# yeyupiaoling/VoiceprintRecognition-Pytorch

Measured on NVIDIA H100. Metric: embeddings/sec (3s@16kHz) ECAPA-TDNN, higher is better.
Workload: dtype f32

## Files before the change

### voiceprintrecognition-pytorch_b200/csrc/api.cu

```cuda
#include <cmath>
#include <cstdarg>
#include <cstdio>
#include <cstdlib>
#include <cstring>
#include <new>
#include <string>
#include <vector>

#include "kernels.cuh"


using namespace vpb;

struct vp_handle {
  int device = 0;
  std::string err;
  float* d_weights = nullptr;
  size_t weights_bytes = 0;
  char* d_arena = nullptr;
  size_t arena_bytes = 0;
  cudaStream_t cap_stream = nullptr;
  bool fe_set = false;
  vp_frontend_desc fe{};
  float* d_window = nullptr;
  double2* d_twiddle = nullptr;
  int* d_mel_start = nullptr;
  int* d_mel_count = nullptr;
  int* d_mel_off = nullptr;
  float* d_mel_w = nullptr;
  float* d_dct = nullptr;
};

struct vp_program {
  vp_handle* h = nullptr;
  std::vector<vp_op> ops;
  std::vector<int> engines;
  size_t ws_bytes = 0, in_floats = 0, out_floats = 0;
  int launches = 0;
  int B = 0;
  cudaGraphExec_t gexec = nullptr;
  const float* g_feats = nullptr;
  float* g_emb = nullptr;
  char* g_arena = nullptr;
  int runs = 0, g_miss = 0;
  bool g_off = false;
  int n_slots = 0;
  size_t arena_need() const { return ws_bytes + (((size_t)n_slots * 4 + 255) & ~(size_t)255); }
  unsigned* slot(int32_t q) const { return q > 0 ? reinterpret_cast<unsigned*>(h->d_arena + ws_bytes) + (q - 1) : nullptr; }
};

static int fail(vp_handle* h, int code, const char* fmt, ...) {
  char buf[512];
  va_list ap;
  va_start(ap, fmt);
  vsnprintf(buf, sizeof(buf), fmt, ap);
  va_end(ap);
  if (h) h->err = buf;
  return code;
}
#define CUDA_TRY(h, expr)                                                                          \
  do {                                                                                             \
    cudaError_t e__ = (expr);                                                                      \
    if (e__ != cudaSuccess) return fail(h, VP_ERR_CUDA, "%s: %s", #expr, cudaGetErrorString(e__)); \
  } while (0)

static const int FPB = 16;

static bool tc16_enabled() {
  static int on = -1;
  if (on < 0) { const char* e = getenv("VPB_TC_F16"); on = (e && e[0] == '0') ? 0 : 1; }
  return on == 1;
}

extern "C" {

static void fill_conv(const vp_program* p, const vp_op& o, const float* feats, float* emb, vpb::ConvParams& c);

int vp_abi_version(void) { return VP_ABI_VERSION; }
int32_t vp_sizeof_op(void) { return (int32_t)sizeof(vp_op); }
int32_t vp_sizeof_frontend_desc(void) { return (int32_t)sizeof(vp_frontend_desc); }

int vp_create(int device, vp_handle** out) {
  if (!out) return VP_ERR_INVALID;
  *out = nullptr;
  int n = 0;
  cudaError_t e = cudaGetDeviceCount(&n);
  if (e != cudaSuccess || device < 0 || device >= n) return VP_ERR_CUDA;
  cudaDeviceProp prop;
  if (cudaGetDeviceProperties(&prop, device) != cudaSuccess) return VP_ERR_CUDA;
// ... 295 lines not shown
      const long long rows = (long long)o.B * o.Tin;
      TRY(check_act_buf(p, "x", o.src, view_floats(rows, o.in_ld, o.in_coff, o.Cin), false, i));
      TRY(check_act_buf(p, "logits", o.src2, view_floats(rows, o.src2_ld, o.src2_coff, o.Cin), false, i));
      if (o.mode != 0 && o.mode != 1) return fail(h, VP_ERR_INVALID, "op %d: asp mode", i);
      TRY(check_act_buf(p, "dst", o.dst, view_floats(o.B, o.out_ld, o.out_coff, (o.mode == 1 ? 1 : 2) * o.Cin), true, i));
      return VP_OK;
    }
    case VP_OP_POOL2D: {
      if (o.Tin < 1 || o.Fin < 1 || o.Tout < 1 || o.Fout < 1 || o.KT < 1 || o.KF < 1 || o.sT < 1 || o.sF < 1 || o.padT < 0 ||
          o.padF < 0 || o.Cin < 4 || (o.Cin & 3) || (o.in_ld & 3) || (o.in_coff & 3) || (o.out_ld & 3) || (o.out_coff & 3) ||
          (o.mode != 0 && o.mode != 1))
        return fail(h, VP_ERR_INVALID, "op %d: pool geometry / alignment", i);
      if ((long long)(o.Tout - 1) * o.sT - o.padT >= o.Tin || (long long)(o.Fout - 1) * o.sF - o.padF >= o.Fin ||
          o.padT >= o.KT || o.padF >= o.KF)
        return fail(h, VP_ERR_INVALID, "op %d: pooling window entirely outside the map", i);
      TRY(check_act_buf(p, "src", o.src, view_floats((long long)o.B * o.Tin * o.Fin, o.in_ld, o.in_coff, o.Cin), false, i));
      TRY(check_act_buf(p, "dst", o.dst, view_floats((long long)o.B * o.Tout * o.Fout, o.out_ld, o.out_coff, o.Cin), true, i));
      return VP_OK;
    }
    case VP_OP_EW: {
      const long long rows = (long long)o.B * o.Tin * o.Fin;
      if (o.mode == VP_EW_PAD_COPY) {
        if (rows < 1 || o.Cin < 1 || o.Cout < o.Cin || (o.Cout & 3) || (o.out_ld & 3) || (o.out_coff & 3))
          return fail(h, VP_ERR_UNSUPPORTED, "op %d: PAD_COPY shape", i);
        TRY(check_act_buf(p, "x", o.src, view_floats(rows, o.in_ld, o.in_coff, o.Cin), false, i));
        TRY(check_act_buf(p, "dst", o.dst, view_floats(rows, o.out_ld, o.out_coff, o.Cout), true, i));
        return VP_OK;
      }
      if (rows < 1 || o.Cin < 4 || (o.Cin & 3) || (o.in_ld & 3) || (o.in_coff & 3) || (o.out_ld & 3) || (o.out_coff & 3))
        return fail(h, VP_ERR_UNSUPPORTED, "op %d: EW alignment", i);
      if (!act_ok(o.act2)) return fail(h, VP_ERR_INVALID, "op %d: activation id", i);
      TRY(check_act_buf(p, "x", o.src, view_floats(rows, o.in_ld, o.in_coff, o.Cin), false, i));
      TRY(check_act_buf(p, "dst", o.dst, view_floats(rows, o.out_ld, o.out_coff, o.Cin), true, i));
      if (o.mode == VP_EW_GATE_RES) {
        if (o.gate != VP_BUF_NONE) TRY(check_act_buf(p, "gate", o.gate, (size_t)o.B * o.Cin, false, i));
        if (o.res != VP_BUF_NONE) {
          if ((o.res_ld & 3) || (o.res_coff & 3)) return fail(h, VP_ERR_UNSUPPORTED, "op %d: res alignment", i);
          TRY(check_act_buf(p, "res", o.res, view_floats(rows, o.res_ld, o.res_coff, o.Cin), false, i));
        }
      } else if (o.mode == VP_EW_AFF) {
        if ((o.src2_ld & 3) || (o.src2_coff & 3) || (o.res_ld & 3) || (o.res_coff & 3)) return fail(h, VP_ERR_UNSUPPORTED, "op %d: AFF alignment", i);
        TRY(check_act_buf(p, "y", o.src2, view_floats(rows, o.src2_ld, o.src2_coff, o.Cin), false, i));
        TRY(check_act_buf(p, "att", o.res, view_floats(rows, o.res_ld, o.res_coff, o.Cin), false, i));
      } else if (o.mode != VP_EW_COPY) {
        return fail(h, VP_ERR_INVALID, "op %d: EW mode", i);
      }
      return VP_OK;
    }
    default:
      return fail(h, VP_ERR_INVALID, "op %d: unknown kind %d", i, o.kind);
  }
}

int vp_program_create(vp_handle* h, const vp_op* ops, int32_t n_ops, size_t ws_bytes, size_t in_floats,
                      size_t out_floats, vp_program** out) {
  if (!h || !ops || n_ops < 1 || !out) return fail(h, VP_ERR_INVALID, "null/empty program");
  if (!h->d_weights) return fail(h, VP_ERR_INVALID, "load weights before creating a program");
  *out = nullptr;
  vp_program* p = new (std::nothrow) vp_program();
  if (!p) return fail(h, VP_ERR_NOMEM, "host alloc");
  p->h = h;
  p->ops.assign(ops, ops + n_ops);
  p->ws_bytes = (ws_bytes + 255) & ~(size_t)255;
  p->in_floats = in_floats;
  p->out_floats = out_floats;
  p->B = p->ops[0].B;
  for (int i = 0; i < n_ops; ++i)
    if (p->ops[i].src == VP_BUF_INPUT) { p->B = p->ops[i].B; break; }
  for (int i = 0; i < n_ops; ++i) {
    int r = validate_op(p, p->ops[i], i);
    if (r != VP_OK) { delete p; return r; }
  }
  p->launches = n_ops;
  p->engines.assign(n_ops, 0);
  for (int i = 0; i < n_ops; ++i) {
    const vp_op& o = p->ops[i];
    if (o.amax_out > p->n_slots) p->n_slots = o.amax_out;
    if (o.amax_in > p->n_slots) p->n_slots = o.amax_in;
  }
  if (p->n_slots > 0) ++p->launches;
  for (int i = 0; i < n_ops; ++i) {
    const vp_op& o = p->ops[i];
    if (o.kind != VP_OP_CONV) continue;
    ConvParams c;
    fill_conv(p, o, nullptr, nullptr, c);
    c.amax_in = o.amax_in > 0 ? reinterpret_cast<const unsigned*>(8) : nullptr;
    const bool ok = conv_tc_supported(c);
    bool ok16 = ok && o.w_tc16_q > 0 && o.tc16_descale > 0.f && conv_tc16_supported(c);
    if (ok16) {
      const int bn = o.tc_bn, nt = (o.Cout + bn - 1) / bn, kb = (c.K + 63) / 64;
      const size_t off = (size_t)(o.w_tc16_q - 1) << 4, bytes = (size_t)nt * kb * 2 * bn * 128;
      if (off + bytes > h->weights_bytes) {
        int r = fail(h, VP_ERR_INVALID, "op %d: fp16 weight image out of range", i);
        delete p;
        return r;
      }
    }
    if ((o.engine == VP_ENGINE_TC && !ok) || (o.engine == VP_ENGINE_TC16 && !ok16)) {
      int r = fail(h, VP_ERR_UNSUPPORTED, "op %d: shape / operands not supported by the requested tensor-core engine", i);
      delete p;
      return r;
    }
    if (o.engine == VP_ENGINE_TC16 || (o.engine == VP_ENGINE_AUTO && ok16 && tc16_enabled())) p->engines[i] = VP_ENGINE_TC16;
    else if (o.engine == VP_ENGINE_TC || (o.engine == VP_ENGINE_AUTO && ok)) p->engines[i] = VP_ENGINE_TC;
    else p->engines[i] = VP_ENGINE_FFMA;
  }
  if (cudaSetDevice(h->device) != cudaSuccess) { delete p; return fail(h, VP_ERR_CUDA, "cudaSetDevice"); }
  if (p->arena_need() > h->arena_bytes) {
    const size_t want = p->arena_need() + (p->arena_need() >> 3);
    cudaDeviceSynchronize();
    cudaFree(h->d_arena);
    h->d_arena = nullptr;
    h->arena_bytes = 0;
    if (cudaMalloc(&h->d_arena, want) != cudaSuccess) {
      cudaGetLastError();
      if (cudaMalloc(&h->d_arena, p->arena_need()) != cudaSuccess) {
        delete p;
        return fail(h, VP_ERR_NOMEM, "workspace of %zu bytes: %s", ws_bytes, cudaGetErrorString(cudaGetLastError()));
      }
      h->arena_bytes = p->arena_need();
    } else {
      h->arena_bytes = want;
    }
  }
  *out = p;
  return VP_OK;
}

void vp_program_destroy(vp_program* p) {
  if (!p) return;
  if (p->gexec) cudaGraphExecDestroy(p->gexec);
  delete p;
}

size_t vp_workspace_bytes(const vp_handle* h) { return h ? h->arena_bytes : 0; }

int32_t vp_program_launches(const vp_program* p) { return p ? p->launches : -1; }

static inline const float* rd(const vp_program* p, int64_t off, const float* in, const float* out) {
  if (off == VP_BUF_NONE) return nullptr;
  if (off == VP_BUF_INPUT) return in;
  if (off == VP_BUF_OUTPUT) return out;
  return reinterpret_cast<const float*>(p->h->d_arena + off);
}
static inline const float* wt(const vp_program* p, int64_t off) {
  return off < 0 ? nullptr : reinterpret_cast<const float*>(reinterpret_cast<const char*>(p->h->d_weights) + off);
}

static void fill_conv(const vp_program* p, const vp_op& o, const float* feats, float* emb, ConvParams& c) {
  c.src = rd(p, o.src, feats, emb);
  c.src2 = o.src2_mode == VP_SRC2_NONE ? nullptr : rd(p, o.src2, feats, emb);
  c.dst = const_cast<float*>(rd(p, o.dst, feats, emb));
  c.sum = const_cast<float*>(rd(p, o.sum, feats, emb)); c.sum_ld = o.sum_ld; c.sum_coff = o.sum_coff;
  c.res = rd(p, o.res, feats, emb); c.gate = rd(p, o.gate, feats, emb); c.ubias = rd(p, o.ubias, feats, emb);
  c.w = wt(p, o.w); c.w_tc = wt(p, o.w_tc); c.tc_bn = o.tc_bn; c.tc_kc = o.tc_kc; c.bias = wt(p, o.bias); c.pre_s = wt(p, o.pre_s); c.pre_h = wt(p, o.pre_h);
  c.post_s = wt(p, o.post_s); c.post_h = wt(p, o.post_h);
  c.B = o.B; c.Tin = o.Tin; c.Fin = o.Fin; c.Cin = o.Cin;
  c.CinTot = o.Cin + (o.src2_mode == VP_SRC2_CONCAT ? o.Cin2 : 0);
  c.in_ld = o.in_ld; c.in_coff = o.in_coff;
  c.src2_mode = o.src2_mode; c.src2_ld = o.src2_ld; c.src2_coff = o.src2_coff;
  c.Tout = o.Tout; c.Fout = o.Fout; c.out_ld = o.out_ld; c.out_coff = o.out_coff;
  c.res_ld = o.res_ld; c.res_coff = o.res_coff;
  c.KT = o.KT; c.KF = o.KF; c.sT = o.sT; c.sF = o.sF; c.dT = o.dT; c.dF = o.dF; c.padT = o.padT; c.padF = o.padF;
  c.pad_mode = o.pad_mode; c.w_ld = o.w_ld; c.pre_relu = o.pre_relu; c.act = o.act; c.act2 = o.act2;
  c.seg_len = o.seg_len; c.n_seg = o.n_seg;
  c.M = o.B * o.Tout * o.Fout; c.N = o.Cout; c.K = o.KT * o.KF * c.CinTot;
  c.amax_out = p->h->d_arena ? p->slot(o.amax_out) : nullptr;
  c.amax_in = p->h->d_arena ? p->slot(o.amax_in) : nullptr;
}

static int run_ops(vp_program* p, const float* feats, float* emb, cudaStream_t st, cudaEvent_t* evs) {
  vp_handle* h = p->h;
  if (p->n_slots > 0) CUDA_TRY(h, cudaMemsetAsync(h->d_arena + p->ws_bytes, 0, (size_t)p->n_slots * 4, st));
  for (size_t i = 0; i < p->ops.size(); ++i) {
    const vp_op& o = p->ops[i];
    if (evs) CUDA_TRY(h, cudaEventRecord(evs[i], st));
    switch (o.kind) {
      case VP_OP_CONV:
      case VP_OP_CONV_C1: {
        ConvParams c;
        fill_conv(p, o, feats, emb, c);
        if (o.kind == VP_OP_CONV_C1) {
          CUDA_TRY(h, launch_conv_c1(c, st));
        } else {
          if (p->engines[i] == VP_ENGINE_TC16)
            CUDA_TRY(h, launch_conv_tc16(c, reinterpret_cast<const float*>(reinterpret_cast<const char*>(h->d_weights) + ((size_t)(o.w_tc16_q - 1) << 4)),
                                         o.tc16_descale, st));
          else if (p->engines[i] == VP_ENGINE_TC) CUDA_TRY(h, launch_conv_tc(c, st));
          else CUDA_TRY(h, launch_conv_ffma(c, st));
        }
        break;
      }
      case VP_OP_COLSTATS: {
        StatsParams s;
        s.src = rd(p, o.src, feats, emb); s.dst = const_cast<float*>(rd(p, o.dst, feats, emb));
        s.B = o.B; s.R = o.Tin * o.Fin; s.C = o.Cin; s.in_ld = o.in_ld; s.in_coff = o.in_coff;
        s.out_ld = o.out_ld; s.out_coff = o.out_coff; s.mode = o.mode; s.seg_len = o.seg_len; s.n_seg = o.n_seg;
        s.eps = o.eps;
        CUDA_TRY(h, launch_colstats(s, st));
        break;
      }
      case VP_OP_ASP_POOL: {
        AspParams a;
        a.x = rd(p, o.src, feats, emb); a.logit = rd(p, o.src2, feats, emb);
        a.dst = const_cast<float*>(rd(p, o.dst, feats, emb));
        a.B = o.B; a.T = o.Tin; a.C = o.Cin; a.x_ld = o.in_ld; a.x_coff = o.in_coff; a.l_ld = o.src2_ld;
        a.l_coff = o.src2_coff; a.out_ld = o.out_ld; a.out_coff = o.out_coff; a.eps = o.eps; a.mean_only = o.mode == 1;
        CUDA_TRY(h, launch_asp_pool(a, st));
        break;
      }
      case VP_OP_POOL2D: {
        PoolParams q;
        q.src = rd(p, o.src, feats, emb); q.dst = const_cast<float*>(rd(p, o.dst, feats, emb));
        q.B = o.B; q.Tin = o.Tin; q.Fin = o.Fin; q.Tout = o.Tout; q.Fout = o.Fout; q.C = o.Cin;
        q.in_ld = o.in_ld; q.in_coff = o.in_coff; q.out_ld = o.out_ld; q.out_coff = o.out_coff;
        q.KT = o.KT; q.KF = o.KF; q.sT = o.sT; q.sF = o.sF; q.padT = o.padT; q.padF = o.padF; q.mode = o.mode;
        q.amax_out = p->slot(o.amax_out);
        CUDA_TRY(h, launch_pool2d(q, st));
        break;
      }
      case VP_OP_EW: {
        EwParams e;
        e.x = rd(p, o.src, feats, emb);
        e.y = o.mode == VP_EW_AFF ? rd(p, o.src2, feats, emb) : nullptr;
        e.att = o.mode == VP_EW_AFF ? rd(p, o.res, feats, emb) : nullptr;
        e.gate = o.mode == VP_EW_GATE_RES ? rd(p, o.gate, feats, emb) : nullptr;
        e.res = o.mode == VP_EW_GATE_RES ? rd(p, o.res, feats, emb) : nullptr;
        e.dst = const_cast<float*>(rd(p, o.dst, feats, emb));
        e.rows = (long long)o.B * o.Tin * o.Fin; e.C = o.Cin; e.rows_per_utt = o.Tin * o.Fin;
// ... 196 lines not shown
```

### voiceprintrecognition-pytorch_b200/csrc/conv_tc.cu

```cuda
#include <cuda_fp16.h>

#include <cstdlib>
#include <type_traits>

#include "kernels.cuh"
#include "wgmma.cuh"

namespace vpb {

namespace tc {

constexpr int BM = 128;
constexpr int BK = 32;
constexpr int A_TILE = BM * BK * 4;
constexpr int CONSUMER_WARPS = 8;
constexpr int CONSUMER_THREADS = CONSUMER_WARPS * 32;
constexpr int PRODUCER_WARPS = 8;
constexpr int PRODUCER_THREADS = PRODUCER_WARPS * 32;
constexpr int NUM_THREADS = CONSUMER_THREADS + PRODUCER_THREADS;
constexpr int ROWS_PER_THREAD = BM * 8 / PRODUCER_THREADS;
constexpr int MAX_BN = 128;
constexpr int MAX_BN_CHUNKED = 64;
constexpr int SMEM_BUDGET = 225 * 1024;

__device__ __forceinline__ uint32_t smem_u32(const void* p) { return (uint32_t)__cvta_generic_to_shared(p); }

__device__ __forceinline__ void mbar_init(uint32_t bar, uint32_t count) {
  asm volatile("mbarrier.init.shared::cta.b64 [%0], %1;" ::"r"(bar), "r"(count));
}
__device__ __forceinline__ void mbar_arrive(uint32_t bar) {
  asm volatile("mbarrier.arrive.shared::cta.b64 _, [%0];" ::"r"(bar) : "memory");
}
__device__ __forceinline__ void mbar_expect_tx(uint32_t bar, uint32_t bytes) {
  asm volatile("mbarrier.arrive.expect_tx.shared::cta.b64 _, [%0], %1;" ::"r"(bar), "r"(bytes) : "memory");
}
__device__ __forceinline__ void mbar_wait(uint32_t bar, uint32_t parity) {
  asm volatile(
      "{\n\t.reg .pred p;\n\t"
      "WAIT_%=:\n\t"
      "mbarrier.try_wait.parity.shared::cta.b64 p, [%0], %1;\n\t"
      "@p bra DONE_%=;\n\t"
      "bra WAIT_%=;\n\t"
      "DONE_%=:\n\t}" ::"r"(bar), "r"(parity)
      : "memory");
}
__device__ __forceinline__ void bulk_copy_g2s(uint32_t dst, const void* src, uint32_t bytes, uint32_t bar) {
  asm volatile("cp.async.bulk.shared::cluster.global.mbarrier::complete_tx::bytes [%0], [%1], %2, [%3];" ::"r"(dst),
               "l"(src), "r"(bytes), "r"(bar)
               : "memory");
}
__device__ __forceinline__ void fence_proxy_async() { asm volatile("fence.proxy.async.shared::cta;" ::: "memory"); }

__device__ __forceinline__ void wgmma_fence() { asm volatile("wgmma.fence.sync.aligned;" ::: "memory"); }
__device__ __forceinline__ void wgmma_commit() { asm volatile("wgmma.commit_group.sync.aligned;" ::: "memory"); }
template <int N>
__device__ __forceinline__ void wgmma_wait() { asm volatile("wgmma.wait_group.sync.aligned %0;" ::"n"(N) : "memory"); }
template <int N>
__device__ __forceinline__ void fence_regs(float (&d)[N]) {
#pragma unroll
  for (int i = 0; i < N; ++i) asm volatile("" : "+f"(d[i])::"memory");
}

__device__ __forceinline__ uint64_t smem_desc(uint32_t addr) {
  return (uint64_t)((addr >> 4) & 0x3FFF) | (1ull << 16) | (64ull << 32) | (1ull << 62);
}
__device__ __forceinline__ float tf32_rna(float x) {
  uint32_t r;
  asm("cvt.rna.tf32.f32 %0, %1;" : "=r"(r) : "f"(x));
  return __uint_as_float(r);
}

template <int BN, bool F16>
__device__ __forceinline__ void mma_tile(float* d, uint32_t a, uint32_t b, uint32_t scale_d) {
  const uint64_t da = smem_desc(a);
  if constexpr (BN == 128) {
    if constexpr (F16) wgmma_f16_n128(d, da, smem_desc(b), scale_d);
    else wgmma_tf32_n128(d, da, smem_desc(b), scale_d);
  } else {
    constexpr int o64 = 0, o32 = o64 + (BN & 64), o16 = o32 + (BN & 32);
    if constexpr ((BN & 64) != 0) {
      if constexpr (F16) wgmma_f16_n64(d + o64 / 2, da, smem_desc(b + o64 * 128), scale_d);
      else wgmma_tf32_n64(d + o64 / 2, da, smem_desc(b + o64 * 128), scale_d);
    }
    if constexpr ((BN & 32) != 0) {
      if constexpr (F16) wgmma_f16_n32(d + o32 / 2, da, smem_desc(b + o32 * 128), scale_d);
      else wgmma_tf32_n32(d + o32 / 2, da, smem_desc(b + o32 * 128), scale_d);
    }
    if constexpr ((BN & 16) != 0) {
      if constexpr (F16) wgmma_f16_n16(d + o16 / 2, da, smem_desc(b + o16 * 128), scale_d);
      else wgmma_tf32_n16(d + o16 / 2, da, smem_desc(b + o16 * 128), scale_d);
    }
  }
}

__device__ __noinline__ float2 act2_slow(float2 v, int act) {
  v.x = apply_act(v.x, act); v.y = apply_act(v.y, act);
  return v;
}

template <int MODE> struct Slot;
template <> struct Slot<0> { float4 v[ROWS_PER_THREAD]; };
template <> struct Slot<1> { float4 v[ROWS_PER_THREAD]; float4 u[ROWS_PER_THREAD]; };
template <> struct Slot<2> { float4 v[ROWS_PER_THREAD]; float4 ps, ph; uint32_t okmask; };
struct SlotH { float4 v[ROWS_PER_THREAD]; float4 w[ROWS_PER_THREAD]; };

struct TcArgs {
  const float* w_tc;
  int BN;
  int stages;
  int m_tiles, n_tiles, k_blocks;
  int kc, n_chunks;
  int debug;
  float descale;
};

template <int MODE, bool F16, int BN>
__global__ void __launch_bounds__(NUM_THREADS, 1) conv_tc_kernel(const __grid_constant__ ConvParams p,
                                                                 const __grid_constant__ TcArgs a) {
  static_assert(!F16 || MODE == 0, "the fp16 split path only implements the plain / concat source mode");
  static_assert(BN % 16 == 0 && BN >= 16 && BN <= MAX_BN, "N tile");
  constexpr bool CHUNKABLE = BN <= MAX_BN_CHUNKED;
  constexpr int BKE = F16 ? 64 : BK;
  constexpr int KPT = F16 ? 8 : 4;
// ... 451 lines not shown
```

### voiceprintrecognition-pytorch_b200/csrc/kernels.cuh

```cuda
#pragma once
#include "common.cuh"

namespace vpb {

struct FrontendParams {
  const float* wave; float* feats; float* partial;
  const float* window; const double2* twiddle;
  const int* mel_start; const int* mel_count; const int* mel_off; const float* mel_w;
  int B, L, T, kind, N, WL, hop, F, remove_dc, power, use_log, fpb, nblk;
  float preemph, log_floor, db_mult;
  float* cta_max;
  int n_pass, radix[12], G;
};
void frontend_plan(FrontendParams& p);

struct MfccParams {
  const float* mel; const float* cta_max; const float* dct; float* feats; float* partial;
  int B, T, M, K, fpb, nblk, n_max;
  float top_db;
};

struct StatsParams {
  const float* src; float* dst;
  int B, R, C, in_ld, in_coff, out_ld, out_coff, mode, seg_len, n_seg;
// ... 1 lines not shown
};

struct AspParams {
  const float* x; const float* logit; float* dst;
  int B, T, C, x_ld, x_coff, l_ld, l_coff, out_ld, out_coff, mean_only;
  float eps;
};

struct EwParams {
  const float* x; const float* y; const float* att; const float* gate; const float* res; float* dst;
  long long rows; int C, rows_per_utt;
  int x_ld, x_coff, y_ld, y_coff, att_ld, att_coff, res_ld, res_coff, out_ld, out_coff, mode, act2;
  int C_out;
  unsigned* amax_out;
};

struct PoolParams {
  const float* src; float* dst;
  int B, Tin, Fin, Tout, Fout, C, in_ld, in_coff, out_ld, out_coff, KT, KF, sT, sF, padT, padF, mode;
  unsigned* amax_out;
};
cudaError_t launch_pool2d(const PoolParams& p, cudaStream_t stream);
cudaError_t launch_cosine_scores(const float* a, const float* b, float* out, int n, int m, int D, cudaStream_t stream);

size_t spectral_scratch_bytes(int n);
int spectral_launches_laplacian();
int spectral_launches_tridiag(int n);
int apply_q_max_rows(int kz);
cudaError_t launch_spectral_laplacian(const float* emb, int n, int D, int n_drop, double* L, void* scratch, cudaStream_t stream);
cudaError_t launch_sym_tridiag(double* A, int n, double* d, double* e, double* tau, void* scratch, cudaStream_t stream);
cudaError_t launch_sym_tridiag_apply_q(const double* A, const double* tau, int n, double* Z, int kz, cudaStream_t stream);

size_t verify_scratch_bytes(int64_t n);
cudaError_t launch_verify_sort(const float* scores, const int32_t* labels, const int32_t* trial, const int32_t* enroll,
                               int64_t n_enroll, int64_t n, void* scratch, cudaStream_t stream);
cudaError_t launch_verify_curve(int64_t n, double p_target, double c_miss, double c_fa, void* scratch, float* sorted_scores,
                                uint8_t* sorted_labels, vp_verify_result* result, cudaStream_t stream);

cudaError_t launch_frontend(const FrontendParams& p, const int* keep, cudaStream_t stream);
cudaError_t launch_frontend_mfcc(const FrontendParams& p, const MfccParams& m, const int* keep, cudaStream_t stream);
cudaError_t launch_frontend_mfcc_mel(const FrontendParams& p, float* max_out, cudaStream_t stream);
cudaError_t launch_frontend_mfcc_finish(const FrontendParams& p, const MfccParams& m, const int* keep, cudaStream_t stream);
size_t frontend_smem_bytes(int N, int WL, int hop, int fpb);
cudaError_t launch_conv_ffma(const ConvParams& p, cudaStream_t stream);
cudaError_t launch_conv_c1(const ConvParams& p, cudaStream_t stream);
cudaError_t launch_colstats(const StatsParams& p, cudaStream_t stream);
cudaError_t launch_asp_pool(const AspParams& p, cudaStream_t stream);
cudaError_t launch_ew(const EwParams& p, cudaStream_t stream);
bool conv_tc_supported(const ConvParams& p);
cudaError_t launch_conv_tc(const ConvParams& p, cudaStream_t stream);
bool conv_tc16_supported(const ConvParams& p);
cudaError_t launch_conv_tc16(const ConvParams& p, const float* w_tc16, float descale, cudaStream_t stream);

}
```

### voiceprintrecognition-pytorch_b200/csrc/wgmma.cuh

```cuda
#pragma once
#include <stdint.h>

namespace vpb {
namespace tc {

__device__ __forceinline__ void wgmma_tf32_n16(float* d, uint64_t a, uint64_t b, uint32_t scale_d) {
  asm volatile(
      "{\n\t.reg .pred p;\n\tsetp.ne.b32 p, %10, 0;\n\t"
      "wgmma.mma_async.sync.aligned.m64n16k8.f32.tf32.tf32 {%0, %1, %2, %3, %4, %5, %6, %7}, %8, %9, p, 1, 1;\n\t}"
      : "+f"(d[0]), "+f"(d[1]), "+f"(d[2]), "+f"(d[3]), "+f"(d[4]), "+f"(d[5]), "+f"(d[6]), "+f"(d[7])
      : "l"(a), "l"(b), "r"(scale_d));
}
__device__ __forceinline__ void wgmma_tf32_n32(float* d, uint64_t a, uint64_t b, uint32_t scale_d) {
  asm volatile(
      "{\n\t.reg .pred p;\n\tsetp.ne.b32 p, %18, 0;\n\t"
      "wgmma.mma_async.sync.aligned.m64n32k8.f32.tf32.tf32 {%0, %1, %2, %3, %4, %5, %6, %7, %8, %9, %10, %11, %12, %13, %14, %15}, %16, %17, p, 1, 1;\n\t}"
      : "+f"(d[0]), "+f"(d[1]), "+f"(d[2]), "+f"(d[3]), "+f"(d[4]), "+f"(d[5]), "+f"(d[6]), "+f"(d[7]), "+f"(d[8]), "+f"(d[9]), "+f"(d[10]), "+f"(d[11]), "+f"(d[12]), "+f"(d[13]), "+f"(d[14]), "+f"(d[15])
      : "l"(a), "l"(b), "r"(scale_d));
}
__device__ __forceinline__ void wgmma_tf32_n64(float* d, uint64_t a, uint64_t b, uint32_t scale_d) {
  asm volatile(
      "{\n\t.reg .pred p;\n\tsetp.ne.b32 p, %34, 0;\n\t"
      "wgmma.mma_async.sync.aligned.m64n64k8.f32.tf32.tf32 {%0, %1, %2, %3, %4, %5, %6, %7, %8, %9, %10, %11, %12, %13, %14, %15, %16, %17, %18, %19, %20, %21, %22, %23, %24, %25, %26, %27, %28, %29, %30, %31}, %32, %33, p, 1, 1;\n\t}"
      : "+f"(d[0]), "+f"(d[1]), "+f"(d[2]), "+f"(d[3]), "+f"(d[4]), "+f"(d[5]), "+f"(d[6]), "+f"(d[7]), "+f"(d[8]), "+f"(d[9]), "+f"(d[10]), "+f"(d[11]), "+f"(d[12]), "+f"(d[13]), "+f"(d[14]), "+f"(d[15]), "+f"(d[16]), "+f"(d[17]), "+f"(d[18]), "+f"(d[19]), "+f"(d[20]), "+f"(d[21]), "+f"(d[22]), "+f"(d[23]), "+f"(d[24]), "+f"(d[25]), "+f"(d[26]), "+f"(d[27]), "+f"(d[28]), "+f"(d[29]), "+f"(d[30]), "+f"(d[31])
      : "l"(a), "l"(b), "r"(scale_d));
}
__device__ __forceinline__ void wgmma_tf32_n128(float* d, uint64_t a, uint64_t b, uint32_t scale_d) {
  asm volatile(
      "{\n\t.reg .pred p;\n\tsetp.ne.b32 p, %66, 0;\n\t"
      "wgmma.mma_async.sync.aligned.m64n128k8.f32.tf32.tf32 {%0, %1, %2, %3, %4, %5, %6, %7, %8, %9, %10, %11, %12, %13, %14, %15, %16, %17, %18, %19, %20, %21, %22, %23, %24, %25, %26, %27, %28, %29, %30, %31, %32, %33, %34, %35, %36, %37, %38, %39, %40, %41, %42, %43, %44, %45, %46, %47, %48, %49, %50, %51, %52, %53, %54, %55, %56, %57, %58, %59, %60, %61, %62, %63}, %64, %65, p, 1, 1;\n\t}"
      : "+f"(d[0]), "+f"(d[1]), "+f"(d[2]), "+f"(d[3]), "+f"(d[4]), "+f"(d[5]), "+f"(d[6]), "+f"(d[7]), "+f"(d[8]), "+f"(d[9]), "+f"(d[10]), "+f"(d[11]), "+f"(d[12]), "+f"(d[13]), "+f"(d[14]), "+f"(d[15]), "+f"(d[16]), "+f"(d[17]), "+f"(d[18]), "+f"(d[19]), "+f"(d[20]), "+f"(d[21]), "+f"(d[22]), "+f"(d[23]), "+f"(d[24]), "+f"(d[25]), "+f"(d[26]), "+f"(d[27]), "+f"(d[28]), "+f"(d[29]), "+f"(d[30]), "+f"(d[31]), "+f"(d[32]), "+f"(d[33]), "+f"(d[34]), "+f"(d[35]), "+f"(d[36]), "+f"(d[37]), "+f"(d[38]), "+f"(d[39]), "+f"(d[40]), "+f"(d[41]), "+f"(d[42]), "+f"(d[43]), "+f"(d[44]), "+f"(d[45]), "+f"(d[46]), "+f"(d[47]), "+f"(d[48]), "+f"(d[49]), "+f"(d[50]), "+f"(d[51]), "+f"(d[52]), "+f"(d[53]), "+f"(d[54]), "+f"(d[55]), "+f"(d[56]), "+f"(d[57]), "+f"(d[58]), "+f"(d[59]), "+f"(d[60]), "+f"(d[61]), "+f"(d[62]), "+f"(d[63])
      : "l"(a), "l"(b), "r"(scale_d));
}
__device__ __forceinline__ void wgmma_f16_n16(float* d, uint64_t a, uint64_t b, uint32_t scale_d) {
  asm volatile(
      "{\n\t.reg .pred p;\n\tsetp.ne.b32 p, %10, 0;\n\t"
      "wgmma.mma_async.sync.aligned.m64n16k16.f32.f16.f16 {%0, %1, %2, %3, %4, %5, %6, %7}, %8, %9, p, 1, 1, 0, 0;\n\t}"
      : "+f"(d[0]), "+f"(d[1]), "+f"(d[2]), "+f"(d[3]), "+f"(d[4]), "+f"(d[5]), "+f"(d[6]), "+f"(d[7])
      : "l"(a), "l"(b), "r"(scale_d));
}
__device__ __forceinline__ void wgmma_f16_n32(float* d, uint64_t a, uint64_t b, uint32_t scale_d) {
  asm volatile(
      "{\n\t.reg .pred p;\n\tsetp.ne.b32 p, %18, 0;\n\t"
      "wgmma.mma_async.sync.aligned.m64n32k16.f32.f16.f16 {%0, %1, %2, %3, %4, %5, %6, %7, %8, %9, %10, %11, %12, %13, %14, %15}, %16, %17, p, 1, 1, 0, 0;\n\t}"
      : "+f"(d[0]), "+f"(d[1]), "+f"(d[2]), "+f"(d[3]), "+f"(d[4]), "+f"(d[5]), "+f"(d[6]), "+f"(d[7]), "+f"(d[8]), "+f"(d[9]), "+f"(d[10]), "+f"(d[11]), "+f"(d[12]), "+f"(d[13]), "+f"(d[14]), "+f"(d[15])
      : "l"(a), "l"(b), "r"(scale_d));
}
__device__ __forceinline__ void wgmma_f16_n64(float* d, uint64_t a, uint64_t b, uint32_t scale_d) {
  asm volatile(
      "{\n\t.reg .pred p;\n\tsetp.ne.b32 p, %34, 0;\n\t"
      "wgmma.mma_async.sync.aligned.m64n64k16.f32.f16.f16 {%0, %1, %2, %3, %4, %5, %6, %7, %8, %9, %10, %11, %12, %13, %14, %15, %16, %17, %18, %19, %20, %21, %22, %23, %24, %25, %26, %27, %28, %29, %30, %31}, %32, %33, p, 1, 1, 0, 0;\n\t}"
      : "+f"(d[0]), "+f"(d[1]), "+f"(d[2]), "+f"(d[3]), "+f"(d[4]), "+f"(d[5]), "+f"(d[6]), "+f"(d[7]), "+f"(d[8]), "+f"(d[9]), "+f"(d[10]), "+f"(d[11]), "+f"(d[12]), "+f"(d[13]), "+f"(d[14]), "+f"(d[15]), "+f"(d[16]), "+f"(d[17]), "+f"(d[18]), "+f"(d[19]), "+f"(d[20]), "+f"(d[21]), "+f"(d[22]), "+f"(d[23]), "+f"(d[24]), "+f"(d[25]), "+f"(d[26]), "+f"(d[27]), "+f"(d[28]), "+f"(d[29]), "+f"(d[30]), "+f"(d[31])
      : "l"(a), "l"(b), "r"(scale_d));
}
__device__ __forceinline__ void wgmma_f16_n128(float* d, uint64_t a, uint64_t b, uint32_t scale_d) {
  asm volatile(
      "{\n\t.reg .pred p;\n\tsetp.ne.b32 p, %66, 0;\n\t"
// ... 8 lines not shown
```

Baseline: 29560.

## Fuse Res2Net split-conv chains into one persistent tensor-core kernel

Detects the Res2Net chain in the op list (a copy of the first split followed by dependent per-split convolutions, each adding the previous output) and replaces it with a single kernel. The kernel keeps a time tile with halo in shared memory, streams each split's weights in with bulk copies, and runs split-tf32 (3xTF32) wgmma with register A operands. It then applies the bias/ReLU/BN epilogue and writes the next split's input back to shared memory. This removes per-split launches and global round-trips between the sequential convs, at the cost of recomputing halo rows and using only one block per batch tile, which may leave SMs idle at small batch.

```diff
diff --git a/voiceprintrecognition-pytorch_b200/csrc/api.cu b/voiceprintrecognition-pytorch_b200/csrc/api.cu
--- a/voiceprintrecognition-pytorch_b200/csrc/api.cu
+++ b/voiceprintrecognition-pytorch_b200/csrc/api.cu
@@ -35,6 +35,7 @@
   vp_handle* h = nullptr;
   std::vector<vp_op> ops;
   std::vector<int> engines;
+  std::vector<int> chain;
   size_t ws_bytes = 0, in_floats = 0, out_floats = 0;
   int launches = 0;
   int B = 0;
@@ -436,6 +437,39 @@
   }
 }
 
+static int find_res2_chain(const vp_program* p, int i) {
+  const vp_op& c = p->ops[i];
+  if (c.kind != VP_OP_EW || c.mode != VP_EW_COPY || c.Fin != 1 || c.src == c.dst) return 0;
+  const int w = c.Cin, n_ops = (int)p->ops.size();
+  int n = 0;
+  for (int j = 1; i + j < n_ops && j <= RES2_MAX_CONVS; ++j) {
+    const vp_op& o = p->ops[i + j];
+    const vp_op& f = p->ops[i + 1];
+    const bool link =
+        o.kind == VP_OP_CONV && p->engines[i + j] == VP_ENGINE_TC && o.B == c.B && o.Cin == w && o.Cout == w &&
+        o.src == c.src && o.in_ld == c.in_ld && o.in_coff == c.in_coff + j * w &&
+        o.dst == c.dst && o.out_ld == c.out_ld && o.out_coff == c.out_coff + j * w &&
+        o.Tin == c.Tin && o.Tout == c.Tin && o.Fin == 1 && o.Fout == 1 && o.KF == 1 && o.sT == 1 && o.sF == 1 &&
+        o.padF == 0 && o.tc_bn == w && o.tc_kc == 0 && o.pre_s < 0 && o.res == VP_BUF_NONE &&
+        o.gate == VP_BUF_NONE && o.ubias == VP_BUF_NONE && o.sum == VP_BUF_NONE && o.act2 == VP_ACT_NONE &&
+        (o.act == VP_ACT_NONE || o.act == VP_ACT_RELU) && o.amax_out == c.amax_out && o.amax_in == 0 &&
+        o.KT == f.KT && o.dT == f.dT && o.padT == f.padT && o.pad_mode == f.pad_mode && o.act == f.act &&
+        (j == 1 ? o.src2_mode == VP_SRC2_NONE
+                : o.src2_mode == VP_SRC2_ADD && o.src2 == c.dst && o.src2_ld == c.out_ld &&
+                      o.src2_coff == c.out_coff + (j - 1) * w);
+    if (!link) break;
+    n = j;
+  }
+  if (n < 1 || !res2_supported(w, n + 1, p->ops[i + 1].KT, p->ops[i + 1].padT)) return 0;
+  if (c.src >= 0 && c.dst >= 0) {
+    const long long rows = (long long)c.B * c.Tin;
+    const long long xs = c.src + 4LL * c.in_coff, xe = c.src + 4LL * ((rows - 1) * c.in_ld + c.in_coff + (n + 1) * w);
+    const long long ys = c.dst + 4LL * c.out_coff, ye = c.dst + 4LL * ((rows - 1) * c.out_ld + c.out_coff + (n + 1) * w);
+    if (xs < ye && ys < xe) return 0;
+  }
+  return n;
+}
+
 int vp_program_create(vp_handle* h, const vp_op* ops, int32_t n_ops, size_t ws_bytes, size_t in_floats,
                       size_t out_floats, vp_program** out) {
   if (!h || !ops || n_ops < 1 || !out) return fail(h, VP_ERR_INVALID, "null/empty program");
@@ -488,6 +522,15 @@
     if (o.engine == VP_ENGINE_TC16 || (o.engine == VP_ENGINE_AUTO && ok16 && tc16_enabled())) p->engines[i] = VP_ENGINE_TC16;
     else if (o.engine == VP_ENGINE_TC || (o.engine == VP_ENGINE_AUTO && ok)) p->engines[i] = VP_ENGINE_TC;
     else p->engines[i] = VP_ENGINE_FFMA;
+  }
+  p->chain.assign(n_ops, 0);
+  for (int i = 0; i < n_ops; ++i) {
+    const int n = find_res2_chain(p, i);
+    if (n == 0) continue;
+    for (int k = i; k < i + n; ++k) p->chain[k] = -1;
+    p->chain[i + n] = n;
+    p->launches -= n;
+    i += n;
   }
   if (cudaSetDevice(h->device) != cudaSuccess) { delete p; return fail(h, VP_ERR_CUDA, "cudaSetDevice"); }
   if (p->arena_need() > h->arena_bytes) {
@@ -553,12 +596,33 @@
   c.amax_in = p->h->d_arena ? p->slot(o.amax_in) : nullptr;
 }
 
+static cudaError_t launch_chain(const vp_program* p, int first, int n, const float* feats, float* emb, cudaStream_t st) {
+  const vp_op& c = p->ops[first];
+  const vp_op& f = p->ops[first + 1];
+  Res2Params r;
+  r.src = rd(p, c.src, feats, emb); r.dst = const_cast<float*>(rd(p, c.dst, feats, emb));
+  for (int j = 0; j < n; ++j) {
+    const vp_op& o = p->ops[first + 1 + j];
+    r.w_tc[j] = wt(p, o.w_tc); r.bias[j] = wt(p, o.bias); r.post_s[j] = wt(p, o.post_s); r.post_h[j] = wt(p, o.post_h);
+  }
+  r.amax_out = p->slot(c.amax_out);
+  r.B = c.B; r.T = c.Tin; r.s = n + 1; r.w = c.Cin;
+  r.in_ld = c.in_ld; r.in_coff = c.in_coff; r.out_ld = c.out_ld; r.out_coff = c.out_coff;
+  r.KT = f.KT; r.dT = f.dT; r.padT = f.padT; r.reflect = f.pad_mode == VP_PAD_REFLECT; r.relu = f.act == VP_ACT_RELU;
+  return launch_res2(r, st);
+}
+
 static int run_ops(vp_program* p, const float* feats, float* emb, cudaStream_t st, cudaEvent_t* evs) {
   vp_handle* h = p->h;
   if (p->n_slots > 0) CUDA_TRY(h, cudaMemsetAsync(h->d_arena + p->ws_bytes, 0, (size_t)p->n_slots * 4, st));
   for (size_t i = 0; i < p->ops.size(); ++i) {
     const vp_op& o = p->ops[i];
     if (evs) CUDA_TRY(h, cudaEventRecord(evs[i], st));
+    if (p->chain[i] < 0) continue;
+    if (p->chain[i] > 0) {
+      CUDA_TRY(h, launch_chain(p, (int)i - p->chain[i], p->chain[i], feats, emb, st));
+      continue;
+    }
     switch (o.kind) {
       case VP_OP_CONV:
       case VP_OP_CONV_C1: {
diff --git a/voiceprintrecognition-pytorch_b200/csrc/conv_tc.cu b/voiceprintrecognition-pytorch_b200/csrc/conv_tc.cu
--- a/voiceprintrecognition-pytorch_b200/csrc/conv_tc.cu
+++ b/voiceprintrecognition-pytorch_b200/csrc/conv_tc.cu
@@ -22,53 +22,6 @@
 constexpr int MAX_BN = 128;
 constexpr int MAX_BN_CHUNKED = 64;
 constexpr int SMEM_BUDGET = 225 * 1024;
-
-__device__ __forceinline__ uint32_t smem_u32(const void* p) { return (uint32_t)__cvta_generic_to_shared(p); }
-
-__device__ __forceinline__ void mbar_init(uint32_t bar, uint32_t count) {
-  asm volatile("mbarrier.init.shared::cta.b64 [%0], %1;" ::"r"(bar), "r"(count));
-}
-__device__ __forceinline__ void mbar_arrive(uint32_t bar) {
-  asm volatile("mbarrier.arrive.shared::cta.b64 _, [%0];" ::"r"(bar) : "memory");
-}
-__device__ __forceinline__ void mbar_expect_tx(uint32_t bar, uint32_t bytes) {
-  asm volatile("mbarrier.arrive.expect_tx.shared::cta.b64 _, [%0], %1;" ::"r"(bar), "r"(bytes) : "memory");
-}
-__device__ __forceinline__ void mbar_wait(uint32_t bar, uint32_t parity) {
-  asm volatile(
-      "{\n\t.reg .pred p;\n\t"
-      "WAIT_%=:\n\t"
-      "mbarrier.try_wait.parity.shared::cta.b64 p, [%0], %1;\n\t"
-      "@p bra DONE_%=;\n\t"
-      "bra WAIT_%=;\n\t"
-      "DONE_%=:\n\t}" ::"r"(bar), "r"(parity)
-      : "memory");
-}
-__device__ __forceinline__ void bulk_copy_g2s(uint32_t dst, const void* src, uint32_t bytes, uint32_t bar) {
-  asm volatile("cp.async.bulk.shared::cluster.global.mbarrier::complete_tx::bytes [%0], [%1], %2, [%3];" ::"r"(dst),
-               "l"(src), "r"(bytes), "r"(bar)
-               : "memory");
-}
-__device__ __forceinline__ void fence_proxy_async() { asm volatile("fence.proxy.async.shared::cta;" ::: "memory"); }
-
-__device__ __forceinline__ void wgmma_fence() { asm volatile("wgmma.fence.sync.aligned;" ::: "memory"); }
-__device__ __forceinline__ void wgmma_commit() { asm volatile("wgmma.commit_group.sync.aligned;" ::: "memory"); }
-template <int N>
-__device__ __forceinline__ void wgmma_wait() { asm volatile("wgmma.wait_group.sync.aligned %0;" ::"n"(N) : "memory"); }
-template <int N>
-__device__ __forceinline__ void fence_regs(float (&d)[N]) {
-#pragma unroll
-  for (int i = 0; i < N; ++i) asm volatile("" : "+f"(d[i])::"memory");
-}
-
-__device__ __forceinline__ uint64_t smem_desc(uint32_t addr) {
-  return (uint64_t)((addr >> 4) & 0x3FFF) | (1ull << 16) | (64ull << 32) | (1ull << 62);
-}
-__device__ __forceinline__ float tf32_rna(float x) {
-  uint32_t r;
-  asm("cvt.rna.tf32.f32 %0, %1;" : "=r"(r) : "f"(x));
-  return __uint_as_float(r);
-}
 
 template <int BN, bool F16>
 __device__ __forceinline__ void mma_tile(float* d, uint32_t a, uint32_t b, uint32_t scale_d) {
diff --git a/voiceprintrecognition-pytorch_b200/csrc/kernels.cuh b/voiceprintrecognition-pytorch_b200/csrc/kernels.cuh
--- a/voiceprintrecognition-pytorch_b200/csrc/kernels.cuh
+++ b/voiceprintrecognition-pytorch_b200/csrc/kernels.cuh
@@ -77,4 +77,17 @@
 bool conv_tc16_supported(const ConvParams& p);
 cudaError_t launch_conv_tc16(const ConvParams& p, const float* w_tc16, float descale, cudaStream_t stream);
 
+constexpr int RES2_MAX_CONVS = 15;
+struct Res2Params {
+  const float* src; float* dst;
+  const float* w_tc[RES2_MAX_CONVS];
+  const float* bias[RES2_MAX_CONVS];
+  const float* post_s[RES2_MAX_CONVS];
+  const float* post_h[RES2_MAX_CONVS];
+  unsigned* amax_out;
+  int B, T, s, w, in_ld, in_coff, out_ld, out_coff, KT, dT, padT, reflect, relu;
+};
+bool res2_supported(int w, int s, int KT, int padT);
+cudaError_t launch_res2(const Res2Params& p, cudaStream_t stream);
+
 }
diff --git a/voiceprintrecognition-pytorch_b200/csrc/res2.cu b/voiceprintrecognition-pytorch_b200/csrc/res2.cu
--- /dev/null
+++ b/voiceprintrecognition-pytorch_b200/csrc/res2.cu
@@ -0,0 +1,252 @@
+#include "kernels.cuh"
+#include "wgmma.cuh"
+
+namespace vpb {
+
+namespace res2 {
+
+constexpr int NWG = 5;
+constexpr int THREADS = NWG * 128;
+constexpr int ROWS = NWG * 64;
+constexpr int SMEM_LIMIT = 227 * 1024;
+
+__host__ __device__ constexpr int k_blocks(int w, int KT) { return (KT * w + 31) / 32; }
+__host__ __device__ constexpr int weight_bytes(int w, int KT) { return k_blocks(w, KT) * 2 * w * 128; }
+__host__ __device__ constexpr int smem_bytes(int w, int KT) { return 1024 + weight_bytes(w, KT) + ROWS * (w + 4) * 4; }
+
+struct Args {
+  Res2Params p;
+  int n_tiles, halo;
+};
+
+template <int BN>
+__device__ __forceinline__ void mma(float* d, const uint32_t (&a)[4], uint32_t b, uint32_t scale_d) {
+  if constexpr (BN == 64) {
+    tc::wgmma_tf32_rA_n64(d, a, tc::smem_desc(b), scale_d);
+  } else {
+    constexpr int o32 = 0, o16 = BN & 32;
+    if constexpr ((BN & 32) != 0) tc::wgmma_tf32_rA_n32(d + o32 / 2, a, tc::smem_desc(b + o32 * 128), scale_d);
+    if constexpr ((BN & 16) != 0) tc::wgmma_tf32_rA_n16(d + o16 / 2, a, tc::smem_desc(b + o16 * 128), scale_d);
+  }
+}
+
+template <int BN>
+__global__ void __launch_bounds__(THREADS, 1) res2_kernel(const __grid_constant__ Args args) {
+  using namespace tc;
+  const Res2Params& p = args.p;
+  constexpr int LDW = BN + 4;
+  pdl_launch_dependents();
+  extern __shared__ uint8_t smem_raw[];
+  __shared__ __align__(8) uint64_t wbar;
+
+  const uint32_t raw = smem_u32(smem_raw);
+  const uint32_t w_s = (raw + 1023u) & ~1023u;
+  const uint32_t wbytes = (uint32_t)weight_bytes(BN, p.KT);
+  float* buf = reinterpret_cast<float*>(smem_raw + (w_s - raw) + wbytes);
+  const uint32_t bar = smem_u32(&wbar);
+
+  const int b = blockIdx.x / args.n_tiles, tile = blockIdx.x - b * args.n_tiles;
+  const int lo = (int)((long long)tile * p.T / args.n_tiles), hi = (int)((long long)(tile + 1) * p.T / args.n_tiles);
+  const int w0 = lo - args.halo > 0 ? lo - args.halo : 0;
+  const int nrows = (hi + args.halo < p.T ? hi + args.halo : p.T) - w0;
+  const float* xu = p.src + (size_t)b * p.T * p.in_ld + p.in_coff;
+  float* yu = p.dst + (size_t)b * p.T * p.out_ld + p.out_coff;
+
+  if (threadIdx.x == 0) {
+    mbar_init(bar, 1);
+    asm volatile("fence.mbarrier_init.release.cluster;" ::: "memory");
+  }
+  __syncthreads();
+  if (threadIdx.x == 0) {
+    mbar_expect_tx(bar, wbytes);
+    bulk_copy_g2s(w_s, p.w_tc[0], wbytes, bar);
+  }
+  pdl_wait();
+
+  float tmax = 0.f;
+  constexpr int C4 = BN / 4;
+  for (int i = threadIdx.x; i < ROWS * C4; i += THREADS) {
+    const int r = i / C4, c = (i - r * C4) * 4;
+    float4 v = make_float4(0.f, 0.f, 0.f, 0.f);
+    if (r < nrows) {
+      const int t = w0 + r;
+      const float* xr = xu + (size_t)t * p.in_ld + c;
+      v = __ldg(reinterpret_cast<const float4*>(xr + BN));
+      if (t >= lo && t < hi) {
+        const float4 y0 = __ldg(reinterpret_cast<const float4*>(xr));
+        *reinterpret_cast<float4*>(yu + (size_t)t * p.out_ld + c) = y0;
+        tmax = amax4(tmax, y0);
+      }
+    }
+    *reinterpret_cast<float4*>(buf + r * LDW + c) = v;
+  }
+  __syncthreads();
+
+  const int wg = threadIdx.x >> 7, lane = threadIdx.x & 31;
+  const int g = lane >> 2, q4 = lane & 3;
+  const int ra = 64 * wg + 16 * ((threadIdx.x >> 5) & 3) + g;
+  const bool active = 64 * wg < nrows;
+  const int ksteps = p.KT * BN / 8;
+  auto load_split = [&](int q, uint32_t (&ah)[4], uint32_t (&al)[4]) {
+    const int k0 = 8 * q, tap = k0 / BN, c0 = k0 - tap * BN + q4;
+    const int sh = tap * p.dT - p.padT;
+    int rr[2];
+    bool ok[2];
+#pragma unroll
+    for (int h = 0; h < 2; ++h) {
+      int t = w0 + ra + 8 * h + sh;
+      ok[h] = true;
+      if (p.reflect) {
+        if (t < 0) t = -t;
+        if (t >= p.T) t = 2 * (p.T - 1) - t;
+      } else {
+        ok[h] = t >= 0 && t < p.T;
+      }
+      int r = t - w0;
+      r = r < 0 ? 0 : (r >= ROWS ? ROWS - 1 : r);
+      rr[h] = r * LDW + c0;
+    }
+    const float x[4] = {ok[0] ? buf[rr[0]] : 0.f, ok[1] ? buf[rr[1]] : 0.f, ok[0] ? buf[rr[0] + 4] : 0.f,
+                        ok[1] ? buf[rr[1] + 4] : 0.f};
+#pragma unroll
+    for (int e = 0; e < 4; ++e) {
+      const float hv = tf32_rna(x[e]);
+      ah[e] = __float_as_uint(hv);
+      al[e] = __float_as_uint(x[e] - hv);
+    }
+  };
+  auto keep = [](uint32_t (&ah)[4], uint32_t (&al)[4]) {
+#pragma unroll
+    for (int e = 0; e < 4; ++e) asm volatile("" : "+r"(ah[e]), "+r"(al[e])::"memory");
+  };
+  for (int j = 1; j < p.s; ++j) {
+    mbar_wait(bar, (uint32_t)(j - 1) & 1u);
+    float acc[BN / 2];
+#pragma unroll
+    for (int i = 0; i < BN / 2; ++i) acc[i] = 0.f;
+    auto step = [&](int q, const uint32_t (&ah)[4], const uint32_t (&al)[4]) {
+      const int k0 = 8 * q;
+      const uint32_t b_hi = w_s + (uint32_t)(k0 >> 5) * (2u * BN * 128u) + (uint32_t)((k0 & 31) * 4);
+      const uint32_t b_lo = b_hi + BN * 128u;
+      wgmma_fence();
+      mma<BN>(acc, al, b_hi, q > 0);
+      mma<BN>(acc, ah, b_lo, 1);
+      mma<BN>(acc, ah, b_hi, 1);
+      wgmma_commit();
+    };
+    if (active) {
+      uint32_t ah0[4], al0[4], ah1[4], al1[4];
+      for (int q = 0; q < ksteps; q += 2) {
+        load_split(q, ah0, al0);
+        step(q, ah0, al0);
+        if (q > 0) { wgmma_wait<1>(); keep(ah1, al1); }
+        load_split(q + 1, ah1, al1);
+        step(q + 1, ah1, al1);
+        wgmma_wait<1>();
+        keep(ah0, al0);
+      }
+      wgmma_wait<0>();
+      keep(ah1, al1);
+      fence_regs(acc);
+    }
+    __syncthreads();
+    if (threadIdx.x == 0 && j + 1 < p.s) {
+      mbar_expect_tx(bar, wbytes);
+      bulk_copy_g2s(w_s, p.w_tc[j], wbytes, bar);
+    }
+    if (active) {
+      const bool last = j + 1 == p.s;
+      const float* bias = p.bias[j - 1];
+      const float* ps = p.post_s[j - 1];
+      const float* ph = p.post_h[j - 1];
+#pragma unroll
+      for (int jj = 0; jj < BN / 8; ++jj) {
+        const int n = 8 * jj + 2 * q4;
+        float2 b2 = make_float2(0.f, 0.f), s2 = make_float2(1.f, 1.f), h2 = b2;
+        if (bias) b2 = __ldg(reinterpret_cast<const float2*>(bias + n));
+        if (ps) {
+          s2 = __ldg(reinterpret_cast<const float2*>(ps + n));
+          h2 = __ldg(reinterpret_cast<const float2*>(ph + n));
+        }
+#pragma unroll
+        for (int h = 0; h < 2; ++h) {
+          const int r = ra + 8 * h;
+          float2 v = make_float2(acc[4 * jj + 2 * h], acc[4 * jj + 2 * h + 1]);
+          v.x = fmaf(v.x, 1.f, b2.x); v.y = fmaf(v.y, 1.f, b2.y);
+          if (p.relu) { v.x = fmaxf(v.x, 0.f); v.y = fmaxf(v.y, 0.f); }
+          if (ps) { v.x = fmaf(v.x, s2.x, h2.x); v.y = fmaf(v.y, s2.y, h2.y); }
+          float2 nxt = make_float2(0.f, 0.f);
+          if (r < nrows) {
+            const int t = w0 + r;
+            if (t >= lo && t < hi) {
+              *reinterpret_cast<float2*>(yu + (size_t)t * p.out_ld + j * BN + n) = v;
+              tmax = fmaxf(tmax, fmaxf(fabsf(v.x), fabsf(v.y)));
+            }
+            if (!last) {
+              const float2 xn = __ldg(reinterpret_cast<const float2*>(xu + (size_t)t * p.in_ld + (j + 1) * BN + n));
+              nxt = make_float2(xn.x + v.x, xn.y + v.y);
+            }
+          }
+          *reinterpret_cast<float2*>(buf + r * LDW + n) = nxt;
+        }
+      }
+    }
+    __syncthreads();
+  }
+  if (p.amax_out) amax_commit(p.amax_out, tmax);
+}
+
+template <int BN>
+static cudaError_t launch_bn(const cudaLaunchConfig_t& cfg, const Args& a) {
+  static PerDeviceSmem once;
+  if (once.need(cfg.dynamicSmemBytes)) {
+    cudaError_t e = cudaFuncSetAttribute(res2_kernel<BN>, cudaFuncAttributeMaxDynamicSharedMemorySize,
+                                         (int)cfg.dynamicSmemBytes);
+    if (e != cudaSuccess) return e;
+    once.set(cfg.dynamicSmemBytes);
+  }
+  return cudaLaunchKernelEx(&cfg, res2_kernel<BN>, a);
+}
+
+}
+
+bool res2_supported(int w, int s, int KT, int padT) {
+  if (w < 16 || w > 64 || (w & 15) || s < 2 || s > RES2_MAX_CONVS + 1 || KT < 1 || padT < 0) return false;
+  if (res2::smem_bytes(w, KT) > res2::SMEM_LIMIT) return false;
+  return 2LL * (s - 1) * padT < res2::ROWS;
+}
+
+cudaError_t launch_res2(const Res2Params& p, cudaStream_t stream) {
+  using namespace res2;
+  if (!res2_supported(p.w, p.s, p.KT, p.padT)) return cudaErrorInvalidConfiguration;
+  Args a;
+  a.p = p;
+  a.halo = (p.s - 1) * p.padT;
+  if (p.T <= ROWS) {
+    a.n_tiles = 1;
+  } else {
+    const int span = ROWS - 2 * a.halo;
+    a.n_tiles = (p.T + span - 1) / span;
+  }
+  cudaLaunchConfig_t cfg{};
+  cfg.gridDim = dim3((unsigned)(p.B * a.n_tiles));
+  cfg.blockDim = dim3(THREADS);
+  cfg.dynamicSmemBytes = (size_t)smem_bytes(p.w, p.KT);
+  cfg.stream = stream;
+  cudaLaunchAttribute attr[1];
+  attr[0].id = cudaLaunchAttributeProgrammaticStreamSerialization;
+  attr[0].val.programmaticStreamSerializationAllowed = pdl_enabled();
+  cfg.attrs = attr;
+  cfg.numAttrs = 1;
+  cudaError_t e;
+  switch (p.w) {
+    case 16: e = launch_bn<16>(cfg, a); break;
+    case 32: e = launch_bn<32>(cfg, a); break;
+    case 48: e = launch_bn<48>(cfg, a); break;
+    default: e = launch_bn<64>(cfg, a); break;
+  }
+  if (e != cudaSuccess) return e;
+  return cudaGetLastError();
+}
+
+}
diff --git a/voiceprintrecognition-pytorch_b200/csrc/wgmma.cuh b/voiceprintrecognition-pytorch_b200/csrc/wgmma.cuh
--- a/voiceprintrecognition-pytorch_b200/csrc/wgmma.cuh
+++ b/voiceprintrecognition-pytorch_b200/csrc/wgmma.cuh
@@ -3,6 +3,75 @@
 
 namespace vpb {
 namespace tc {
+
+__device__ __forceinline__ uint32_t smem_u32(const void* p) { return (uint32_t)__cvta_generic_to_shared(p); }
+
+__device__ __forceinline__ void mbar_init(uint32_t bar, uint32_t count) {
+  asm volatile("mbarrier.init.shared::cta.b64 [%0], %1;" ::"r"(bar), "r"(count));
+}
+__device__ __forceinline__ void mbar_arrive(uint32_t bar) {
+  asm volatile("mbarrier.arrive.shared::cta.b64 _, [%0];" ::"r"(bar) : "memory");
+}
+__device__ __forceinline__ void mbar_expect_tx(uint32_t bar, uint32_t bytes) {
+  asm volatile("mbarrier.arrive.expect_tx.shared::cta.b64 _, [%0], %1;" ::"r"(bar), "r"(bytes) : "memory");
+}
+__device__ __forceinline__ void mbar_wait(uint32_t bar, uint32_t parity) {
+  asm volatile(
+      "{\n\t.reg .pred p;\n\t"
+      "WAIT_%=:\n\t"
+      "mbarrier.try_wait.parity.shared::cta.b64 p, [%0], %1;\n\t"
+      "@p bra DONE_%=;\n\t"
+      "bra WAIT_%=;\n\t"
+      "DONE_%=:\n\t}" ::"r"(bar), "r"(parity)
+      : "memory");
+}
+__device__ __forceinline__ void bulk_copy_g2s(uint32_t dst, const void* src, uint32_t bytes, uint32_t bar) {
+  asm volatile("cp.async.bulk.shared::cluster.global.mbarrier::complete_tx::bytes [%0], [%1], %2, [%3];" ::"r"(dst),
+               "l"(src), "r"(bytes), "r"(bar)
+               : "memory");
+}
+__device__ __forceinline__ void fence_proxy_async() { asm volatile("fence.proxy.async.shared::cta;" ::: "memory"); }
+
+__device__ __forceinline__ void wgmma_fence() { asm volatile("wgmma.fence.sync.aligned;" ::: "memory"); }
+__device__ __forceinline__ void wgmma_commit() { asm volatile("wgmma.commit_group.sync.aligned;" ::: "memory"); }
+template <int N>
+__device__ __forceinline__ void wgmma_wait() { asm volatile("wgmma.wait_group.sync.aligned %0;" ::"n"(N) : "memory"); }
+template <int N>
+__device__ __forceinline__ void fence_regs(float (&d)[N]) {
+#pragma unroll
+  for (int i = 0; i < N; ++i) asm volatile("" : "+f"(d[i])::"memory");
+}
+
+__device__ __forceinline__ uint64_t smem_desc(uint32_t addr) {
+  return (uint64_t)((addr >> 4) & 0x3FFF) | (1ull << 16) | (64ull << 32) | (1ull << 62);
+}
+__device__ __forceinline__ float tf32_rna(float x) {
+  uint32_t r;
+  asm("cvt.rna.tf32.f32 %0, %1;" : "=r"(r) : "f"(x));
+  return __uint_as_float(r);
+}
+
+__device__ __forceinline__ void wgmma_tf32_rA_n16(float* d, const uint32_t (&a)[4], uint64_t b, uint32_t scale_d) {
+  asm volatile(
+      "{\n\t.reg .pred p;\n\tsetp.ne.b32 p, %13, 0;\n\t"
+      "wgmma.mma_async.sync.aligned.m64n16k8.f32.tf32.tf32 {%0, %1, %2, %3, %4, %5, %6, %7}, {%8, %9, %10, %11}, %12, p, 1, 1;\n\t}"
+      : "+f"(d[0]), "+f"(d[1]), "+f"(d[2]), "+f"(d[3]), "+f"(d[4]), "+f"(d[5]), "+f"(d[6]), "+f"(d[7])
+      : "r"(a[0]), "r"(a[1]), "r"(a[2]), "r"(a[3]), "l"(b), "r"(scale_d));
+}
+__device__ __forceinline__ void wgmma_tf32_rA_n32(float* d, const uint32_t (&a)[4], uint64_t b, uint32_t scale_d) {
+  asm volatile(
+      "{\n\t.reg .pred p;\n\tsetp.ne.b32 p, %21, 0;\n\t"
+      "wgmma.mma_async.sync.aligned.m64n32k8.f32.tf32.tf32 {%0, %1, %2, %3, %4, %5, %6, %7, %8, %9, %10, %11, %12, %13, %14, %15}, {%16, %17, %18, %19}, %20, p, 1, 1;\n\t}"
+      : "+f"(d[0]), "+f"(d[1]), "+f"(d[2]), "+f"(d[3]), "+f"(d[4]), "+f"(d[5]), "+f"(d[6]), "+f"(d[7]), "+f"(d[8]), "+f"(d[9]), "+f"(d[10]), "+f"(d[11]), "+f"(d[12]), "+f"(d[13]), "+f"(d[14]), "+f"(d[15])
+      : "r"(a[0]), "r"(a[1]), "r"(a[2]), "r"(a[3]), "l"(b), "r"(scale_d));
+}
+__device__ __forceinline__ void wgmma_tf32_rA_n64(float* d, const uint32_t (&a)[4], uint64_t b, uint32_t scale_d) {
+  asm volatile(
+      "{\n\t.reg .pred p;\n\tsetp.ne.b32 p, %37, 0;\n\t"
+      "wgmma.mma_async.sync.aligned.m64n64k8.f32.tf32.tf32 {%0, %1, %2, %3, %4, %5, %6, %7, %8, %9, %10, %11, %12, %13, %14, %15, %16, %17, %18, %19, %20, %21, %22, %23, %24, %25, %26, %27, %28, %29, %30, %31}, {%32, %33, %34, %35}, %36, p, 1, 1;\n\t}"
+      : "+f"(d[0]), "+f"(d[1]), "+f"(d[2]), "+f"(d[3]), "+f"(d[4]), "+f"(d[5]), "+f"(d[6]), "+f"(d[7]), "+f"(d[8]), "+f"(d[9]), "+f"(d[10]), "+f"(d[11]), "+f"(d[12]), "+f"(d[13]), "+f"(d[14]), "+f"(d[15]), "+f"(d[16]), "+f"(d[17]), "+f"(d[18]), "+f"(d[19]), "+f"(d[20]), "+f"(d[21]), "+f"(d[22]), "+f"(d[23]), "+f"(d[24]), "+f"(d[25]), "+f"(d[26]), "+f"(d[27]), "+f"(d[28]), "+f"(d[29]), "+f"(d[30]), "+f"(d[31])
+      : "r"(a[0]), "r"(a[1]), "r"(a[2]), "r"(a[3]), "l"(b), "r"(scale_d));
+}
 
 __device__ __forceinline__ void wgmma_tf32_n16(float* d, uint64_t a, uint64_t b, uint32_t scale_d) {
   asm volatile(
```

Result: faster. 30350, median of 6 (+2.7%).
